# alpenlabs/dv-pari

Hardware: AMD Instinct MI355X
Metric: R1CS constraints/sec (prove) (higher is better)
Workload: dtype u32; 1 GPU; Proof::prove, synthetic dense R1CS, 2^20 constraints (BASELINE config #4); log2_constraints=20, n_wires=1048576, msm_pairs_per_proof=6291456, witness=resident in HBM, entry=dvp_prove_dev (Proof::prove with the witness resident), proofs_in_flight=1

## Files before the change

### dv-pari_amd/_native.py

```python
import ctypes as C
import os

import numpy as np

_HERE = os.path.dirname(os.path.abspath(__file__))
LIB_PATH = os.environ.get("DVP_LIB") or os.path.join(_HERE, "libdvpari_hip.so")

if not os.environ.get("DVP_NO_TORCH_PRELOAD"):
    try:
        import torch
    except Exception:
        pass

if not os.path.exists(LIB_PATH):
    raise ImportError(
        f"{LIB_PATH} is missing: build it with `python -c 'import __graft_entry__ as g; g.build()'` "
        "(hipcc --offload-arch=gfx950).  dv-pari_amd has no CPU fallback."
    )
lib = C.CDLL(LIB_PATH)

vp, u32, u64p, u8p, sz = C.c_void_p, C.c_uint32, C.c_void_p, C.c_void_p, C.c_size_t


class DlogReport(C.Structure):
# ... 158 lines not shown
    "dvp_prove_dev": (C.c_int, [vp, vp, u8p, vp]),
    "dvp_prove_begin": (C.c_int, [vp, vp, vp]),
    "dvp_prove_begin_partial": (C.c_int, [vp, vp, C.c_int, vp]),
    "dvp_prover_extend_count": (u32, [vp]),
    "dvp_prove_extend_vectors": (C.c_int, [vp, u32, vp]),
    "dvp_prover_extended_ptr": (C.c_int, [vp, u32, C.POINTER(vp)]),
    "dvp_prove_quotient": (C.c_int, [vp, vp]),
    "dvp_prove_mark_extended": (C.c_int, [vp, u32]),
    "dvp_prover_msm_size": (C.c_size_t, [vp, C.c_int]),
    "dvp_prover_msm_plan": (C.c_int, [vp, C.c_int, C.POINTER(C.c_int), C.POINTER(C.c_int)]),
    "dvp_prover_msm_table_bytes": (C.c_uint64, [vp, C.c_int, C.POINTER(C.c_int)]),
    "dvp_prover_set_table_budget": (C.c_int, [vp, C.c_uint64]),
    "dvp_prover_msm_coverage": (C.c_int, [vp, C.c_int, C.POINTER(C.c_size_t), C.POINTER(C.c_size_t), C.POINTER(C.c_int)]),
    "dvp_table_plan": (C.c_int, [sz, sz, C.c_uint64, C.POINTER(C.c_size_t * 2), C.POINTER(C.c_uint64 * 2)]),
    "dvp_aff_share_plan": (C.c_int, [C.c_longlong, u32, C.c_uint64, C.c_uint64, C.c_uint64]),
    "dvp_prover_msm_partial": (C.c_int, [vp, C.c_int, sz, sz, vp, vp, vp]),
    "dvp_prove_challenge": (C.c_int, [vp, vp, vp, vp]),
    "dvp_prove_challenge_partial": (C.c_int, [vp, vp, vp, C.c_size_t, C.c_size_t, C.c_size_t, C.c_size_t, vp, vp]),
    "dvp_prove_challenge_finish": (C.c_int, [vp, vp, C.c_uint32, C.c_size_t, C.c_size_t, vp]),
    "dvp_prove_finish": (C.c_int, [vp, vp, vp, u8p, vp]),
    "dvp_prover_debug_read": (C.c_int, [vp, C.c_char_p, u64p, sz]),
    "dvp_prover_debug_transcript_dev": (C.c_int, [vp, u8p, u64p, u32, u64p, u64p]),
    "dvp_prover_debug_force_alpha": (C.c_int, [vp, u64p]),
    "dvp_prover_domains": (C.c_int, [vp, u64p, u64p]),
    "dvp_prover_domain_tables": (C.c_int, [vp, C.c_int, u64p, u64p]),
    "dvp_ecfft_domain_tables": (C.c_int, [vp, C.c_int, u64p, u64p]),
    "dvp_file_fr_vec_write": (C.c_int, [C.c_char_p, u64p, sz]),
    "dvp_file_fr_vec_read": (C.c_int, [C.c_char_p, u64p, sz, C.POINTER(C.c_size_t)]),
    "dvp_file_point_vec_write": (C.c_int, [C.c_char_p, u8p, sz]),
    "dvp_file_point_vec_read": (C.c_int, [C.c_char_p, u8p, sz, C.POINTER(C.c_size_t)]),
# ... 144 lines not shown
```

### dv-pari_amd/csrc/capi.cpp

```cpp
#include "common.h"

#include <atomic>
#include <map>
#include <mutex>
#include <string>
#include <vector>
#include <cstring>
#include <cstdlib>
#include <climits>
#include <cxxabi.h>

namespace dvp {
thread_local int64_t g_last_error_index = -1;
thread_local hipError_t g_last_hip_error = hipSuccess;

bool g_prof_enabled = false;
static unsigned g_prof_mask = ~0u;
static std::mutex g_prof_mu;
static double g_prof_ms[PROF_NSLOTS] = {0};
static uint64_t g_prof_n[PROF_NSLOTS] = {0};
struct Pending { int slot; hipEvent_t e0, e1; uint64_t key; };
struct Shape { double ms = 0; uint64_t n = 0; };
static std::map<uint64_t, Shape> g_prof_round0;
static std::vector<Pending> g_prof_pending;
// ... 20 lines not shown
      g_prof_n[p.slot] += (p.slot == PROF_MSM_AFFINE_REST && p.key) ? p.key : 1;
      if (p.slot == PROF_MSM_ACCUM_AFFINE && p.key) { Shape& sh = g_prof_round0[p.key]; sh.ms += ms; sh.n += 1; }
    }
    (void)hipEventDestroy(p.e0);
    (void)hipEventDestroy(p.e1);
  }
  g_prof_pending.clear();
}

static std::atomic<uint64_t> g_host_waits[2];
void count_host_wait(int kind) { g_host_waits[kind & 1].fetch_add(1, std::memory_order_relaxed); }
static std::atomic<uint64_t> g_later_rounds[2];
void count_later_round(bool dense) { g_later_rounds[dense ? 1 : 0].fetch_add(1, std::memory_order_relaxed); }
static std::atomic<uint64_t> g_rounds_inv[2];
void count_round_inv(bool shared) { g_rounds_inv[shared ? 1 : 0].fetch_add(1, std::memory_order_relaxed); }

struct Census {
  std::mutex mu;
  std::map<std::string, LaunchCounter*> by_name;
};
static Census& census() {
  static Census* c = new Census;
  return *c;
}
LaunchCounter* census_register(const char* file, const char* tag_type) {
  int st = 0;
  char* dm = abi::__cxa_demangle(tag_type ? tag_type : "", nullptr, nullptr, &st);
  std::string v = (st == 0 && dm) ? dm : (tag_type ? tag_type : "");
  free(dm);
  for (size_t at; (at = v.find("(anonymous namespace)::")) != std::string::npos;) v.erase(at, 23);
// ... 43 lines not shown
    {"DVP_MSM_AFF_BMIN", &Tune::msm_aff_bmin},
    {"DVP_MSM_AFF_SHARE_INV", &Tune::msm_aff_share_inv},
    {"DVP_MSM_AFF_SHARE_MIN", &Tune::msm_aff_share_min},
    {"DVP_MSM_AFF_BMAX", &Tune::msm_aff_bmax},
    {"DVP_ECFFT_RADIX4", &Tune::ecfft_radix4},
    {"DVP_ECFFT_FOLD", &Tune::ecfft_fold},
    {"DVP_MSM_ACCUM_FAST", &Tune::msm_accum_fast},
    {"DVP_MSM_TAIL_GROUPS", &Tune::msm_tail_groups},
    {"DVP_MSM_ACCUM_HEX_MAX", &Tune::msm_accum_hex_max},
    {"DVP_GF_INV_TABS", &Tune::gf_inv_tabs},
    {"DVP_MSM_ACCUM_QUAD_MAX", &Tune::msm_accum_quad_max},
    {"DVP_MSM_BUCKET_PAIRS_MAX", &Tune::msm_bucket_pairs_max},
    {"DVP_MSM_SORT_FUSED", &Tune::msm_sort_fused},
    {"DVP_MSM_ROUND_PIPELINE", &Tune::msm_round_pipeline},
    {"DVP_MSM_ROUND_DENSE", &Tune::msm_round_dense},
    {"DVP_MSM_HEX_MAX", &Tune::msm_hex_max},
    {"DVP_MSM_QUAD_MAX", &Tune::msm_quad_max},
    {"DVP_MSM_FIXED_MIN", &Tune::msm_fixed_min},
    {"DVP_FR_BI_SHAPE", &Tune::fr_bi_shape},
    {"DVP_HORNER_MAX_PUB", &Tune::horner_max_pub},
    {"DVP_PROVE_HOST_TRANSCRIPT", &Tune::prove_host_transcript},
    {"DVP_TABLE_BUDGET_BYTES", &Tune::table_budget_bytes},
    {"DVP_MSM_TABLE_REFUSE", &Tune::msm_table_refuse},
    {"DVP_POINTS_MUL_W", &Tune::points_mul_w},
    {"DVP_MSM_SEG_PIECE", &Tune::msm_seg_piece},
    {"DVP_CIRCUIT_HASH_WINDOW", &Tune::circuit_hash_window},
    {"DVP_MSM_ALIGNED_SIGNED", &Tune::msm_aligned_signed},
    {"DVP_FR_DIGEST_WINDOW", &Tune::fr_digest_window},
};
static_assert(sizeof(Tune) == sizeof(kKnobs) / sizeof(kKnobs[0]) * sizeof(long long), "every field of Tune needs exactly one row of kKnobs");
// ... 54 lines not shown
extern "C" void dvp_profile_enable(int on) {
  dvp::g_prof_mask = on == 2 ? (1u << dvp::PROF_MSM_ACCUM_AFFINE) : ~0u;
  dvp::g_prof_enabled = on != 0;
}
extern "C" void dvp_profile_reset(void) {
  dvp::prof_collect();
  std::lock_guard<std::mutex> g(dvp::g_prof_mu);
  for (int i = 0; i < dvp::PROF_NSLOTS; ++i) { dvp::g_prof_ms[i] = 0; dvp::g_prof_n[i] = 0; }
  dvp::g_prof_round0.clear();
  dvp::g_host_waits[0] = 0;
  dvp::g_host_waits[1] = 0;
  dvp::g_later_rounds[0] = 0;
  dvp::g_later_rounds[1] = 0;
  dvp::g_rounds_inv[0] = 0;
  dvp::g_rounds_inv[1] = 0;
  dvp::Census& c = dvp::census();
  std::lock_guard<std::mutex> gc(c.mu);
  for (auto& e : c.by_name) e.second->n.store(0, std::memory_order_relaxed);
}
extern "C" int dvp_debug_launch_names(char* buf, size_t cap) {
  dvp::Census& c = dvp::census();
  std::lock_guard<std::mutex> g(c.mu);
  std::string all;
  for (auto& e : c.by_name) { all += e.first; all += '\n'; }
  if (buf && cap) {
    const size_t k = all.size() < cap - 1 ? all.size() : cap - 1;
    memcpy(buf, all.data(), k);
    buf[k] = 0;
  }
  return (int)(all.size() + 1);
// ... 12 lines not shown
extern "C" int dvp_profile_read(const char* name, double* total_ms, uint64_t* launches) {
  if (!name || !total_ms || !launches) return DVP_EINVAL;
  if (!strcmp(name, "host_waits_stream") || !strcmp(name, "host_waits_side")) {
    *total_ms = 0;
    *launches = dvp::g_host_waits[name[11] == 's' && name[12] == 'i' ? 1 : 0].load();
    return DVP_OK;
  }
  if (!strcmp(name, "later_rounds_word") || !strcmp(name, "later_rounds_dense")) {
    *total_ms = 0;
    *launches = dvp::g_later_rounds[name[13] == 'd' ? 1 : 0].load();
    return DVP_OK;
  }
  if (!strcmp(name, "rounds_inv_private") || !strcmp(name, "rounds_inv_shared")) {
    *total_ms = 0;
    *launches = dvp::g_rounds_inv[name[11] == 's' ? 1 : 0].load();
    return DVP_OK;
  }
  if (!strncmp(name, "launch:", 7)) {
    dvp::Census& c = dvp::census();
    std::lock_guard<std::mutex> g(c.mu);
    auto it = c.by_name.find(name + 7);
    if (it == c.by_name.end()) return DVP_EINVAL;
    *total_ms = 0;
    *launches = it->second->n.load(std::memory_order_relaxed);
    return DVP_OK;
  }
  dvp::prof_collect();
  std::lock_guard<std::mutex> g(dvp::g_prof_mu);
  for (int i = 0; i < dvp::PROF_NSLOTS; ++i)
    if (!strcmp(name, dvp::kProfNames[i])) { *total_ms = dvp::g_prof_ms[i]; *launches = dvp::g_prof_n[i]; return DVP_OK; }
// ... 46 lines not shown
```

### dv-pari_amd/csrc/common.h

```cpp
#pragma once
#include <hip/hip_runtime.h>
#include <stdint.h>
#include <stdio.h>
#include <string.h>

#include <algorithm>
#include <atomic>
#include <mutex>
#include <typeinfo>
#include <vector>

#include "../../include/dvpari_internal.h"
#include "fr.cuh"
#include "host_api.h"

namespace dvp {

extern thread_local hipError_t g_last_hip_error;

inline int hip_fail(hipError_t e, const char* what, const char* file, int line) {
  g_last_hip_error = e;
  fprintf(stderr, "[dvpari] HIP error %d (%s) at %s:%d: %s\n", (int)e, hipGetErrorString(e), file, line, what);
  if (e == hipErrorOutOfMemory) {
    (void)hipGetLastError();
// ... 179 lines not shown
  long long msm_aff_bmin = 8;
  long long msm_aff_share_inv = 2;
  long long msm_aff_share_min = 0;
  long long msm_aff_bmax = 136;
  long long ecfft_radix4 = 3;
  long long ecfft_fold = 1;
  long long msm_accum_fast = 1;
  long long msm_tail_groups = 1;
  long long msm_accum_hex_max = -1;
  long long gf_inv_tabs = 1;
  long long msm_accum_quad_max = 0;
  long long msm_bucket_pairs_max = 12;
  long long msm_sort_fused = 1;
  long long msm_round_pipeline = 2;
  long long msm_round_dense = 0;
  long long msm_hex_max = -1;
  long long msm_quad_max = 0;
  long long msm_fixed_min = 1ll << 16;
  long long fr_bi_shape = 6;
  long long horner_max_pub = -1;
  long long prove_host_transcript = 0;
  long long table_budget_bytes = -1;
  long long msm_table_refuse = 0;
  long long points_mul_w = 3;
  long long msm_seg_piece = 4;
  long long circuit_hash_window = 0;
  long long msm_aligned_signed = 1;
  long long fr_digest_window = 0;
};
Tune& tune();
// ... 5 lines not shown

enum ProfSlot { PROF_MSM_ACCUM_AFFINE = 0, PROF_MSM_TOTAL, PROF_EXTEND_TOTAL, PROF_PROVE_TOTAL, PROF_MSM_AFFINE_REST, PROF_MSM_SORT, PROF_MSM_TAIL, PROF_NSLOTS };
extern bool g_prof_enabled;
struct ProfScope {
  int slot;
  hipStream_t st;
  hipEvent_t e0 = nullptr, e1 = nullptr;
  uint64_t key = 0;
  ProfScope(int slot_, hipStream_t st_, uint64_t key_ = 0);
  void stop();
};
void prof_collect();
void count_host_wait(int kind);
void count_later_round(bool dense);
void count_round_inv(bool shared);

struct LaunchCounter {
  std::atomic<uint64_t> n{0};
};
LaunchCounter* census_register(const char* file, const char* tag_type);
template <auto K>
struct LaunchTag {};
template <auto K>
struct LaunchSite {
  static LaunchCounter* const counter;
};
template <auto K>
LaunchCounter* const LaunchSite<K>::counter = census_register(__BASE_FILE__, typeid(LaunchTag<K>).name());
template <auto K>
struct Launch;
// ... 11 lines not shown
```

### dv-pari_amd/csrc/msm.hip

```cpp
#include <algorithm>
#include <cstdlib>
#include <cstring>
#include <atomic>
#include <chrono>
#include <mutex>
#include <type_traits>
#include <vector>

#include "common.h"
#include "k233.cuh"
#include "tau.cuh"
#include "codec.cuh"
#include "host_api.h"
#include "msm_recode.cuh"
#include "msm_scan.cuh"
#include "msm_sort.cuh"
#include "msm_table.cuh"
#include "msm_reduce.cuh"
#include "msm_rounds.cuh"
#include "msm_merge.cuh"

namespace dvp {

static std::mutex g_wave_trace_mu;
// ... 235 lines not shown
  else if (per_key >= 8) f(std::integral_constant<int, 16>{});
  else f(std::integral_constant<int, 4>{});
}

struct MsmLayout {
  FxBits fb;
  bool fused1;
  uint32_t fx_S, fx_nblk, fx_nch;
  size_t sort_cells, affA_n, affB_n;
  bool affine_mode;
  size_t aff_min, e_est;
  int ra_plan;
  bool pipelined, side_stream;
  bool dense;
  size_t desc_at[41], desc_n;
  size_t rest_cap;
  uint32_t tail_groups;
  size_t bytes;
  bool sort_done_by_mscan() const { return pipelined && !side_stream; }
};
struct MsmBuffers {
  unsigned long long* err;
  uint32_t *d_max, *rest_n;
  uint16_t *digits, *plo, *hist16;
  uint32_t *digits32, *pid, *phist, *pbase, *ctot, *pstart, *cstart, *pcount, *chunk_off;
  uint32_t *cnt, *off, *ntask, *toff, *cnt2, *off2, *bsum, *items, *rest_list;
  Ld *bufA, *bufB, *bkt, *tail;
  Aff *affA, *affB;
  Gf* prefix;
  uint32_t* gdesc;
  uint32_t* rp;
  uint32_t* bsum2;
};
static MsmBuffers msm_carve(size_t n, const MsmPlan& p, const MsmFixedCtx* fx, const MsmLayout& L, void* base, size_t* bytes = nullptr) {
  Carver c{(uintptr_t)base};
  MsmBuffers b;
  const uint32_t FX_NP = L.fb.np();
  const size_t keys4 = ((size_t)p.nkeys + 1) * 4;
  b.err = c.take<unsigned long long>(32);
  b.d_max = (uint32_t*)(b.err + 1);
  b.rest_n = b.d_max + 1;
  b.digits = c.take<uint16_t>(fx ? 16 : (size_t)p.W * n * 2);
  b.digits32 = c.take<uint32_t>(fx && !L.fused1 ? p.e_max * 4 : 16);
// ... 1 lines not shown
  b.pid = c.take<uint32_t>(fx ? p.e_max * 4 : 16);
  for (uint32_t** r : {&b.phist, &b.pbase}) *r = c.take<uint32_t>(fx ? (size_t)L.fx_nblk * FX_NP * 4 : 16);
  b.ctot = c.take<uint32_t>(fx ? (size_t)FX_NP * L.fx_nch * 4 : 16);
  b.pstart = c.take<uint32_t>((FX_NP_MAX + 1) * 4 * 3);
  b.cstart = b.pstart + FX_NP_MAX + 1;
  b.pcount = b.cstart + FX_NP_MAX + 1;
  for (uint32_t** r : {&b.cnt, &b.off, &b.ntask, &b.toff, &b.cnt2, &b.off2}) *r = c.take<uint32_t>(keys4);
  b.bsum = c.take<uint32_t>(((size_t)p.nkeys / SCAN_BLK + 8) * 4);
  b.items = c.take<uint32_t>((p.e_max + (size_t)p.nkeys + 2) * 4);
  b.hist16 = c.take<uint16_t>(L.sort_cells * 2);
  b.chunk_off = c.take<uint32_t>(L.sort_cells * 4);
  b.bufA = c.take<Ld>(p.t1_max * sizeof(Ld));
  b.bufB = c.take<Ld>(p.t2_max * sizeof(Ld));
  b.affA = c.take<Aff>(L.affine_mode ? L.affA_n * sizeof(Aff) : 16);
  b.affB = c.take<Aff>(L.affine_mode ? L.affB_n * sizeof(Aff) : 16);
  b.prefix = c.take<Gf>(L.affine_mode ? (L.affA_n + 256) * sizeof(Gf) : 16);
  b.gdesc = c.take<uint32_t>(L.affine_mode ? L.desc_n * sizeof(uint32_t) : 16);
  b.rp = c.take<uint32_t>(L.pipelined ? (size_t)L.ra_plan * 2 * keys4 : 16);
  b.bsum2 = c.take<uint32_t>(((size_t)((L.ra_plan > 0 ? L.ra_plan : 1) + 1) * ((size_t)p.nkeys / SCAN_BLK + 1) + 8) * 4);
  b.bkt = c.take<Ld>((size_t)p.nkeys * sizeof(Ld));
  b.rest_list = c.take<uint32_t>(L.rest_cap * 4);
  b.tail = c.take<Ld>(((size_t)2 * p.W * p.c + 1 + 2 * (size_t)L.tail_groups) * sizeof(Ld));
  if (bytes) *bytes = c.o;
  return b;
}
static MsmLayout msm_layout(size_t n, const MsmPlan& p, const MsmFixedCtx* fx, const Tune& tn) {
  MsmLayout L{};
  L.fb = fx ? fx->bits() : FxBits{0, 0};
  L.fused1 = fx && fx->signed_digits && tn.msm_sort_fused != 0;
  L.fx_S = L.fused1 ? (FX_CHUNK / (uint32_t)p.W > 0 ? FX_CHUNK / (uint32_t)p.W : 1u) : 0u;
  L.fx_nblk = L.fused1 ? cdiv(n, L.fx_S) : cdiv(p.e_max, FX_CHUNK);
// ... 5 lines not shown
  L.aff_min = (size_t)(tn.msm_aff_min > 0 ? tn.msm_aff_min : 1);
  L.e_est = (size_t)n * (size_t)((fx && fx->signed_digits) ? p.W : (234 + p.c - 1) / p.c);
  while (L.affine_mode && L.ra_plan < 40 && (L.e_est >> (L.ra_plan + 1)) >= L.aff_min) ++L.ra_plan;
  L.pipelined = L.affine_mode && tn.msm_round_pipeline != 0 && L.ra_plan >= 2 && L.e_est >= 4 * (size_t)p.nkeys;
  L.side_stream = L.pipelined && tn.msm_round_pipeline == 1;
  L.dense = L.pipelined && tn.msm_round_dense != 0;
  L.desc_n = L.affA_n + 64;
  if (L.pipelined) {
    size_t cap_r = p.e_max + p.nkeys, at = 0;
    for (int r = 0; r < L.ra_plan; ++r) {
      const size_t out_max = cap_r / 2 + p.nkeys + 1;
      if (r >= 1) { L.desc_at[r] = at; at += (L.dense ? 2 : 1) * (out_max + 64); }
      cap_r = out_max;
    }
    if (at > L.desc_n) L.desc_n = at;
  }
  L.rest_cap = (size_t)p.nkeys + 2 + (p.e_max + (size_t)p.nkeys) / (size_t)(p.K > 0 ? p.K : 1);
  L.tail_groups = ((uint32_t)(p.W * p.c) + 15u) / 16u;
  (void)msm_carve(n, p, fx, L, nullptr, &L.bytes);
  return L;
}

static int msm_acquire_workspace(int dev, hipStream_t st, int ws_slots, size_t bytes, std::unique_lock<std::mutex>& g, MsmWorkspace** out) {
  int ws_slot = 0;
  for (int pass = 0; pass < 2 && !g.owns_lock(); ++pass)
    for (int sl = 0; sl < ws_slots && !g.owns_lock(); ++sl) {
      g = std::unique_lock<std::mutex>(g_ws_dev[dev][sl].mu, std::try_to_lock);
      if (g.owns_lock() && pass == 0 && g_ws_dev[dev][sl].busy_for(st)) g.unlock();
      if (g.owns_lock()) ws_slot = sl;
    }
// ... 207 lines not shown
    if (e != ~0ull) {
      g_last_error_index = (int64_t)(e & 0xffffffffull);
      return DVP_EINVAL;
    }
    return DVP_OK;
  }
};

static bool aff_share_plan(long long mode, uint32_t tpb, uint64_t planned, uint64_t share_min, uint64_t chip_full) {
  if (tpb != 128 && tpb != 256) return false;
  if (mode == 1) return true;
  if (mode != 2) return false;
  return planned >= (share_min ? share_min : chip_full);
}

struct PairRounds {
  const MsmRun& m;
  uint32_t *pc[3], *po[3];
  int cur = 0;
  const Aff* pts_in;
  size_t cap;
  int launched = 0, ra = 0;
  uint32_t max_cnt = 0;
  uint32_t aff_tpb = 0, aff_lds = 0, aff_cap = 0, aff_bmax_only = 0, aff_bmax = 0, aff_bmin = 0, wt_cap = 0;
  unsigned long long* wt_buf = nullptr;
  std::unique_lock<std::mutex> heavy;
  explicit PairRounds(const MsmRun& m_)
      : m(m_), pc{m_.b.cnt, m_.b.ntask, m_.b.cnt2}, po{m_.b.off, m_.b.toff, m_.b.off2}, pts_in(m_.bases0), cap(m_.p.e_max + m_.p.nkeys) {}
  uint32_t* rc(int r) const { return r == 0 ? m.b.cnt : m.b.rp + (size_t)(2 * (r - 1)) * ((size_t)m.p.nkeys + 1); }
  uint32_t* ro(int r) const { return r == 0 ? m.b.off : m.b.rp + (size_t)(2 * (r - 1) + 1) * ((size_t)m.p.nkeys + 1); }
// ... 36 lines not shown
    const size_t out_max = cap / 2 + nk + 1;
    Aff* outp = (r & 1) ? b.affB : b.affA;
    const uint32_t r_max = cdiv(cdiv(out_max, aff_cap), aff_bmax_only);
    const uint32_t grid = r_max * (aff_cap / aff_tpb) + 1;
    const bool share = aff_share_plan(m.tn.msm_aff_share_inv, aff_tpb, (uint64_t)(L.e_est >> (r + 1)),
                                      m.tn.msm_aff_share_min > 0 ? (uint64_t)m.tn.msm_aff_share_min : 0, (uint64_t)aff_cap * aff_bmin);
    const uint32_t bmax_arg = aff_bmax | (share ? AFF_SHARE_INV : 0u);
    ProfScope ps0(r == 0 ? PROF_MSM_ACCUM_AFFINE : -1, st, (uint64_t)m.n);
    WaveTrace wt{wt_buf, wt_cap, g_wave_trace_tag.fetch_add(wt_buf ? 1u : 0u)};
    with_bool(r == 0, [&](auto first) {
      with_bool(wt.buf != nullptr, [&](auto trace) {
        with_bool(r > 0 && L.dense, [&](auto dense) {
          constexpr bool FIRST = decltype(first)::value, TRACE = decltype(trace)::value, DENSE = decltype(dense)::value;
          if constexpr (!(FIRST && DENSE))
            DVP_LAUNCH((k_affine_round<FIRST, TRACE, DENSE>), dim3(grid), dim3(aff_tpb), aff_lds, st, pts_in, (const uint2*)(const void*)dsc, d_total,
                       aff_cap, bmax_arg, m.Tsq, b.prefix, outp, FIRST ? m.sign_mask : 0u, wt);
        });
      });
    });
    ps0.stop();
    if (r > 0) count_later_round(L.dense);
    count_round_inv(share);
    if (MsmCapture* c = m.cap; c && r < (int)CAPTURE_MAX_ROUNDS) {
      const bool dense_r = r > 0 && L.dense;
      const size_t pts_n = std::min(out_max, (r & 1) ? L.affB_n : L.affA_n);
      const size_t desc_n = r == 0 ? 0 : (L.pipelined ? (dense_r ? 2 : 1) * (out_max + 64) : std::min(out_max, L.desc_n));
      MsmCapture::Round& cr = c->rounds[r];
      cr.ocnt = c->grab(L.pipelined ? rc(r + 1) : pc[nxt], (size_t)nk * 4, st);
      cr.ooff = c->grab(L.pipelined ? ro(r + 1) : po[nxt], ((size_t)nk + 1) * 4, st);
      cr.desc = c->grab(dsc, desc_n * 4, st);
      cr.pts = c->grab(outp, pts_n * sizeof(Aff), st);
      c->hdr[CH_SHARE + r] = share ? 1u : 0u;
      c->nrounds = (uint32_t)r + 1;
    }
    pts_in = outp;
    cap = out_max;
    if (!L.pipelined) cur = nxt;
    return DVP_OK;
  }
  int begin() {
    const MsmLayout& L = m.L;
    if (m.ws_slots > 1 && L.affine_mode) {
      HeavyGate& hg = g_heavy[m.dev];
      heavy = std::unique_lock<std::mutex>(hg.mu);
      if (hg.last && hg.last != m.ws->ev_heavy) DVP_HIP(hipStreamWaitEvent(m.st, hg.last, 0));
    }
    if (L.affine_mode && (L.e_est >> 1) >= L.aff_min && L.e_est >= 4 * (size_t)m.p.nkeys) {
      DVP_TRY(run(0));
      launched = 1;
    }
    DVP_HIP(hipStreamSynchronize(m.ws->aux));
    count_host_wait(launched ? 1 : 0);
    max_cnt = *m.ws->pinned;
    if (L.affine_mode)
// ... 9 lines not shown
  int finish() {
    int r_evt = -1;
    if (heavy.owns_lock() && ra > 0) {
      const size_t gate_min = m.tn.msm_gate_min > 0 ? (size_t)m.tn.msm_gate_min : 1;
      r_evt = 0;
      while (r_evt + 1 < ra && (m.L.e_est >> (r_evt + 2)) >= gate_min) ++r_evt;
    }
    if (r_evt >= 0 && r_evt < launched) DVP_TRY(gate_event());
    int r = launched;
    if (r == 0 && ra > 0) {
      DVP_TRY(run(0));
      if (r_evt == 0) DVP_TRY(gate_event());
      r = 1;
    }
    ProfScope ps_rest(ra > r ? PROF_MSM_AFFINE_REST : -1, m.st, (uint64_t)(ra > r ? ra - r : 0));
    for (; r < ra; ++r) {
      DVP_TRY(run(r));
      if (r == r_evt) DVP_TRY(gate_event());
    }
    ps_rest.stop();
    if (m.L.pipelined) {
      pc[0] = rc(ra);
      po[0] = ro(ra);
      cur = 0;
    }
    if (heavy.owns_lock()) heavy.unlock();
    return DVP_OK;
  }
};

// ... 235 lines not shown
}
void msm_fixed_destroy(MsmFixedCtx* c) {
  if (!c) return;
  if (c->table) (void)hipFree(c->table);
  delete c;
}
int msm_fixed_dev(const MsmFixedCtx* c, const void* d_scalars, const void* d_inf, uint32_t lo, uint32_t hi, const MsmOut& out, hipStream_t st) {
  if (!c || lo > hi || hi > c->n_total) return DVP_EINVAL;
  return msm_core(d_scalars, nullptr, d_inf, hi - lo, c, lo, out, st);
}

}

using namespace dvp;

extern "C" int dvp_aff_share_plan(long long mode, uint32_t tpb, uint64_t planned, uint64_t share_min, uint64_t chip_full) {
  return aff_share_plan(mode, tpb, planned, share_min, chip_full) ? 1 : 0;
}

static size_t table_max_prefix(size_t total, uint64_t budget, size_t fixed_min, uint64_t* bytes) {
  *bytes = 0;
  if (total == 0 || total < fixed_min || total >= ((size_t)1 << 27)) return 0;
  size_t n = total;
  for (int it = 0; it < 64 && n > 0; ++it) {
    const uint64_t per = (uint64_t)msm_fixed_rows_for(n) * sizeof(Aff);
    const uint64_t fit = budget / per;
    if (fit >= n) break;
    n = (size_t)fit;
  }
  while (n > 0 && (uint64_t)msm_fixed_rows_for(n) * n * sizeof(Aff) > budget) --n;
// ... 111 lines not shown
```

### dv-pari_amd/csrc/msm_rounds.cuh

```cuda
#pragma once
#include "common.h"
#include "k233.cuh"
#include "msm_scan.cuh"
#include "msm_reduce.cuh"

namespace dvp {

constexpr uint32_t AFF_NONE = 0xffffffffu;
constexpr uint32_t DESC_PAIR = 0x80000000u;

__global__ void __launch_bounds__(256)
k_post_sort(uint32_t* __restrict__ items, const uint32_t* __restrict__ cnt, const uint32_t* __restrict__ off , uint32_t nkeys,
            uint32_t* __restrict__ ocnt, uint32_t* __restrict__ ooff , uint32_t* __restrict__ d_max) {
  const uint32_t k = blockIdx.x * blockDim.x + threadIdx.x;
  uint32_t m = 0;
  if (k <= nkeys) {
    const uint32_t o = off[k];
    ooff[k] = o >> 1;
    if (k < nkeys) {
      const uint32_t c = cnt[k];
      if (c & 1) items[o + c] = AFF_NONE;
      ocnt[k] = (c + 1) >> 1;
      m = c;
    }
// ... 166 lines not shown
    case 1: __builtin_amdgcn_s_setprio(1); break;
    default: __builtin_amdgcn_s_setprio(2); break;
  }
}
constexpr uint32_t AFF_BMAX = 136;
__device__ __forceinline__ uint32_t aff_slots_per_thread(uint32_t total, uint32_t cap, uint32_t bmax_bmin) {
  const uint32_t bmax = bmax_bmin & 0xffu, bmin = (bmax_bmin >> 8) & 0xffu;
  const uint32_t units = (total + cap - 1) / cap;
  const uint32_t R = (units + bmax - 1) / bmax;
  const uint32_t B = R ? (units + R - 1) / R : 1;
  return B < bmin ? bmin : B;
}
constexpr uint32_t AFF_SHARE_INV = 1u << 16;
constexpr uint32_t AFF_X_SLOT_BYTES = 2048;
constexpr uint32_t aff_exchange_bytes(uint32_t waves) { return waves == 4 ? 6 * AFF_X_SLOT_BYTES : waves == 2 ? 3 * AFF_X_SLOT_BYTES : 0; }
constexpr uint32_t AFF_INV_SPREAD = 256;
__device__ __forceinline__ void aff_x_put(uint32_t lane_addr, uint32_t slot, const Gf& v) {
  const uint32_t a = lane_addr + slot * AFF_X_SLOT_BYTES;
  gf_lds_st(a, (gf_u32x4){v.w[0], v.w[1], v.w[2], v.w[3]});
  gf_lds_st(a + 1024, (gf_u32x4){v.w[4], v.w[5], v.w[6], v.w[7]});
}
__device__ __forceinline__ Gf aff_x_get(uint32_t lane_addr, uint32_t slot) {
  const uint32_t a = lane_addr + slot * AFF_X_SLOT_BYTES;
  const gf_u32x4 lo = gf_lds_ld(a), hi = gf_lds_ld(a + 1024);
  Gf r;
  r.w[0] = lo.x; r.w[1] = lo.y; r.w[2] = lo.z; r.w[3] = lo.w;
  r.w[4] = hi.x; r.w[5] = hi.y; r.w[6] = hi.z; r.w[7] = hi.w;
  return r;
}
struct WaveTrace {
// ... 14 lines not shown
    for (int i = 0; i < 8; ++i) y.w[i] = gf_andxor(neg, x.w[i], y.w[i]);
  }
}
template <bool FIRST, bool DENSE>
__device__ __forceinline__ AffSlot aff_ld_desc(const uint2* __restrict__ desc, int k, int B, uint32_t sk, uint32_t lim) {
  const bool ok = k >= 0 && k < B && sk < lim;
  const uint32_t at = ok ? sk : 0u;
  const uint2 d = (FIRST || DENSE) ? desc[at] : make_uint2(((const uint32_t*)desc)[at], 0u);
  if (FIRST) return AffSlot{ok ? d.x : AFF_NONE, ok ? d.y : AFF_NONE, 0u};
  const uint32_t a = d.x & ~DESC_PAIR;
  return AffSlot{ok ? a : AFF_NONE, (ok && (d.x & DESC_PAIR)) ? a + 1 : AFF_NONE, d.y};
}
template <bool FIRST, bool TRACE = false, bool DENSE = false>
__global__ void __launch_bounds__(EC_TPB) __attribute__((amdgpu_waves_per_eu(3, 3)))
k_affine_round(const Aff* __restrict__ pts, const uint2* __restrict__ desc, const uint32_t* __restrict__ total_ptr ,
               uint32_t cap, uint32_t bmax, GfSqrTables T, Gf* __restrict__ prefix, Aff* __restrict__ out, uint32_t sign_mask, WaveTrace wt) {
  extern __shared__ char lds_raw[];
  unsigned long long tr_t0 = 0, tr_c0 = 0, tr_t1 = 0, tr_t2 = 0;
  uint32_t tr_inverted = 0;
  if (TRACE) { tr_t0 = wall_clock64(); tr_c0 = clock64(); }
  GfLdsK L = gf_ldsk_init(lds_raw);
#if AFF_PRIO
  const uint32_t wslot = __builtin_amdgcn_s_getreg(((4 - 1) << 11) | 4);
#endif
  const uint32_t sm = FIRST ? sign_mask : 0u;
  auto ldx = [&](uint32_t v) -> Gf { return pts[v & ~sm].x; };
  auto ldp = [&](uint32_t v, Gf& x, Gf& y) { aff_ld_point<FIRST>(pts, sm, v, x, y); };
  const uint32_t total = *total_ptr;
  const int B = (int)aff_slots_per_thread(total, cap, bmax);
  const uint32_t nthr = (total + B - 1) / B;
  const uint32_t tid = blockIdx.x * blockDim.x + threadIdx.x;
  const bool share = (bmax & AFF_SHARE_INV) != 0 && blockDim.x > 64;
  if (share ? blockIdx.x * blockDim.x >= nthr : tid >= nthr) return;
  const bool wave_live = __builtin_amdgcn_readfirstlane(tid & ~63u) < nthr;
  const uint32_t lim = tid < nthr ? total : 0u;
  auto ld_desc = [&](int k, uint32_t sk) -> AffSlot { return aff_ld_desc<FIRST, DENSE>(desc, k, B, sk, lim); };
  const Gf one = gf_one();
  Gf run = one;
  if (wave_live) {
    uint32_t sk = tid, sp = tid;
    AffSlot d0 = ld_desc(0, sk);
    sk += nthr;
    AffSlot d1 = ld_desc(1, sk);
    sk += nthr;
    Gf xa, ya, xb, yb;
    {
      const bool p = d0.b != AFF_NONE;
      ldp(p ? d0.a : 0u, xa, ya);
      ldp(p ? d0.b : 0u, xb, yb);
    }
#pragma unroll 1
    for (int k = 0; k < B; ++k) {
#if AFF_PRIO
      aff_set_prio(wslot + (uint32_t)k);
#endif
      const bool pair = d0.b != AFF_NONE;
      Gf den = gf_add(xa, xb), num = gf_add(ya, yb);
      const bool ainf = aff_or8(xa) == 0u, binf = aff_or8(xb) == 0u;
      const bool rare = pair & (ainf | binf | (aff_or8(den) == 0u));
      bool dbl = false;
      den.w[0] |= pair ? 0u : 1u;
      if (__any(rare)) {
        if (rare) {
          dbl = !ainf & !binf & (aff_or8(num) == 0u);
          den = dbl ? xa : one;
          num = dbl ? ya : gf_zero();
        }
      }
      const AffSlot d2 = ld_desc(k + 2, sk);
      sk += nthr;
      {
        const bool p = d1.b != AFF_NONE;
        if (!DENSE || __any(p)) {
          ldp(p ? d1.a : 0u, xa, ya);
          ldp(p ? d1.b : 0u, xb, yb);
        }
      }
      if (!DENSE || __any(pair)) {
        Gf np, nrun;
        gf_mul2(num, den, run, L, np, nrun);
        if (__any(rare)) {
          if (rare) np.w[7] |= dbl ? AFF_W7_DBL : AFF_W7_SKIP;
        }
        if (pair) prefix[sp] = np;
        run = nrun;
      }
      sp += nthr;
      d0 = d1;
      d1 = d2;
    }
// ... 4 lines not shown
  const uint32_t inverting = (blockIdx.x / AFF_INV_SPREAD) & (W - 1);
  Gf inv = run;
  if (share) {
    if (TRACE) tr_inverted = w == inverting ? 3u : 2u;
    aff_x_put(xa, w, run);
    __syncthreads();
    if (W == 4) {
      if ((w & 1u) == 0) aff_x_put(xa, 4 + (w >> 1), gf_mul(run, aff_x_get(xa, w + 1), L));
      __syncthreads();
    }
    if (w == inverting) {
      __builtin_amdgcn_s_setprio(3);
      inv = gf_mul(aff_x_get(xa, W == 4 ? 4 : 0), aff_x_get(xa, W == 4 ? 5 : 1), L);
    }
  }
  if (!share || w == inverting) inv = gf_inv_fast(inv, T, L);
  if (share) {
    if (w == inverting) {
      if (W == 4) {
        Gf ia, ib;
        gf_mul2(aff_x_get(xa, 5), aff_x_get(xa, 4), inv, L, ia, ib);
        aff_x_put(xa, 4, ia);
        aff_x_put(xa, 5, ib);
      } else {
        aff_x_put(xa, 2, inv);
      }
      __builtin_amdgcn_s_setprio(0);
    }
    __syncthreads();
    inv = gf_mul(aff_x_get(xa, W == 4 ? 4 + (w >> 1) : 2), aff_x_get(xa, w ^ 1u), L);
  }
  if (TRACE) tr_t2 = wall_clock64();
  if (wave_live) {
    uint32_t sp = (uint32_t)(B - 1) * nthr + tid, sk = sp;
    auto ld_slot = [&](const AffSlot& e, uint32_t s, Gf& x1, Gf& y1, Gf& x2, Gf& pre) {
      const bool pair = e.b != AFF_NONE;
      ldp(e.a != AFF_NONE ? e.a : 0u, x1, y1);
      x2 = ldx(pair ? e.b : 0u);
      pre = prefix[pair ? s : 0u];
    };
    AffSlot e0 = ld_desc(B - 1, sk);
    sk -= nthr;
    AffSlot e1 = ld_desc(B - 2, sk);
    sk -= nthr;
    Gf px, py, qx, pre;
    ld_slot(e0, sp, px, py, qx, pre);
#pragma unroll 1
    for (int k = B - 1; k >= 0; --k) {
#if AFF_PRIO
      aff_set_prio(wslot + (uint32_t)k);
#endif
      const bool pair = e0.b != AFF_NONE, flagged = pair & (pre.w[7] > AFF_W7_MASK);
      const uint32_t sidx = DENSE ? e0.o : sp;
// ... 36 lines not shown
      } else if (e0.a != AFF_NONE && !pair) {
        out[sidx].x = px;
        out[sidx].y = py;
      }
      sp -= nthr;
      e0 = e1;
      e1 = e2;
      px = npx;
      py = npy;
      pre = npre;
    }
  }
#if AFF_PRIO
  __builtin_amdgcn_s_setprio(0);
#endif
  if (TRACE) {
    const unsigned long long t3 = wall_clock64(), c3 = clock64();
    if ((threadIdx.x & 63u) == 0) {
      const unsigned long long i = atomicAdd(wt.buf, 1ull);
      if (i < wt.cap) {
        unsigned long long* r = wt.buf + 8 + 8 * i;
        r[0] = tr_t0; r[1] = tr_t1; r[2] = tr_t2; r[3] = t3;
        r[4] = tr_c0; r[5] = c3;
        r[6] = (unsigned long long)__builtin_amdgcn_s_getreg((31 << 11) | 4) | ((unsigned long long)__builtin_amdgcn_s_getreg((31 << 11) | 20) << 32);
        r[7] = (unsigned long long)blockIdx.x | ((unsigned long long)wt.tag << 32) | ((unsigned long long)(uint32_t)B << 48) | ((unsigned long long)(threadIdx.x >> 6) << 56) |
               ((unsigned long long)tr_inverted << 60);
      }
    }
  }
}
// ... 38 lines not shown
```

### include/dvpari_internal.h

```cpp
#ifndef DVPARI_INTERNAL_H
#define DVPARI_INTERNAL_H

#include "dvpari.h"

#ifdef __cplusplus
extern "C" {
#endif

int dvp_tune_set(const char* name, long long value);
int dvp_tune_get(const char* name, long long* value);
void dvp_tune_reset(void);

void dvp_profile_enable(int on);
void dvp_profile_reset(void);
int dvp_profile_read(const char* name, double* total_ms, uint64_t* launches);
int dvp_debug_launch_names(char* buf, size_t cap);
int dvp_debug_msm_rest_len(uint32_t* n);

int dvp_debug_msm_capture_arm(size_t arena_bytes);
int dvp_debug_msm_capture_fetch(void* out, size_t cap_bytes, size_t* need);
int dvp_debug_msm_enc(dvp_msm_ctx* ctx, const uint64_t* scalars, const uint64_t* bases_xy, size_t lo, size_t hi, uint64_t out_xy[8],
                      int* out_is_infinity, uint8_t out_enc[30]);

int dvp_profile_round0_shapes(uint64_t* pairs, double* total_ms, uint64_t* launches, int cap);

int dvp_ubench_gf_mul(int reps, double* products_per_s);
int dvp_ubench_fr_mul(int reps, double* muladds_per_s);
int dvp_ubench_points_check(const void* d_xy, const void* d_inf, const void* d_enc, size_t n, void* d_scratch, int reps,
                            double* check_ms, double* decode_ms);
int dvp_ubench_points_mul(const void* d_scalars, const void* d_xy, size_t n, void* d_scratch, int reps, double* mul_ms, double* mulgen_ms);
int dvp_debug_wave_trace(void* d_buf, uint32_t n_records);
int dvp_ubench_gather(const void* d_table, size_t table_bytes, int reps, double* gathers_per_s);
int dvp_prover_msm_table_ptr(const dvp_prover* p, int which, const void** d_table, uint64_t* bytes);

int dvp_table_plan(size_t size0, size_t size1, uint64_t budget_bytes, size_t covered[2], uint64_t bytes[2]);

int dvp_aff_share_plan(long long mode, uint32_t tpb, uint64_t planned, uint64_t share_min, uint64_t chip_full);

int dvp_debug_recode_signed(const uint64_t* scalars, size_t n, int c_bits, uint32_t* out_words, int* windows);

int dvp_debug_recode_tnaf(const uint64_t* scalars, size_t n, int w, int8_t* digits, int* n_digits, int32_t* alpha );

int dvp_setup_scalars(const uint64_t tau[4], const uint64_t delta[4], const uint64_t epsilon[4], uint32_t log2_m, uint32_t n_public,
                      uint32_t n_rows, uint32_t n_wires, const uint64_t* coeffs, uint32_t n_coeffs, const uint32_t* const row_ptr[3],
                      const uint32_t* const wire_ids[3], const uint32_t* const coeff_ids[3], uint64_t* out_scalars, size_t out_cap);

int dvp_setup_cache_dir_ex(const uint64_t tau[4], const uint64_t delta[4], const uint64_t epsilon[4], const char* cache_dir,
                           uint32_t n_public, int write_precomputes, uint64_t* out_scalars, size_t out_cap, uint32_t* out_n_wires,
                           uint32_t* out_log2_m);

int dvp_prover_debug_transcript_dev(dvp_prover* p, const uint8_t commit_p[30], const uint64_t* public_inputs, uint32_t n_public,
                                    uint64_t out_alpha[4], uint64_t out_neg_z_alpha[4]);
// ... 90 lines not shown
```

Before: 59.75 million constraints/s.

## Fuse later affine MSM reduction rounds into one persistent kernel launch

Adds a fused path that runs all remaining affine bucket-reduction rounds inside a single k_affine_round launch. Each workgroup takes a key range found by binary search over the round offsets and loops through the rounds, with only block-level barriers and fences between rounds. This is meant to remove per-round launch overhead and the grid-wide serialization between small later rounds. It relies on each workgroup's key range staying self-contained across rounds, uses an extra output buffer, and may load-balance poorly when buckets are skewed.

```diff
diff --git a/dv-pari_amd/_native.py b/dv-pari_amd/_native.py
--- a/dv-pari_amd/_native.py
+++ b/dv-pari_amd/_native.py
@@ -196,6 +196,7 @@
     "dvp_prover_msm_coverage": (C.c_int, [vp, C.c_int, C.POINTER(C.c_size_t), C.POINTER(C.c_size_t), C.POINTER(C.c_int)]),
     "dvp_table_plan": (C.c_int, [sz, sz, C.c_uint64, C.POINTER(C.c_size_t * 2), C.POINTER(C.c_uint64 * 2)]),
     "dvp_aff_share_plan": (C.c_int, [C.c_longlong, u32, C.c_uint64, C.c_uint64, C.c_uint64]),
+    "dvp_round_fuse_plan": (C.c_int, [C.c_longlong, C.c_int, C.c_int, C.c_int, C.c_uint64, C.c_uint64, C.c_uint64]),
     "dvp_prover_msm_partial": (C.c_int, [vp, C.c_int, sz, sz, vp, vp, vp]),
     "dvp_prove_challenge": (C.c_int, [vp, vp, vp, vp]),
     "dvp_prove_challenge_partial": (C.c_int, [vp, vp, vp, C.c_size_t, C.c_size_t, C.c_size_t, C.c_size_t, vp, vp]),
diff --git a/dv-pari_amd/csrc/capi.cpp b/dv-pari_amd/csrc/capi.cpp
--- a/dv-pari_amd/csrc/capi.cpp
+++ b/dv-pari_amd/csrc/capi.cpp
@@ -58,6 +58,8 @@
 void count_later_round(bool dense) { g_later_rounds[dense ? 1 : 0].fetch_add(1, std::memory_order_relaxed); }
 static std::atomic<uint64_t> g_rounds_inv[2];
 void count_round_inv(bool shared) { g_rounds_inv[shared ? 1 : 0].fetch_add(1, std::memory_order_relaxed); }
+static std::atomic<uint64_t> g_rounds_fused;
+void count_round_fused() { g_rounds_fused.fetch_add(1, std::memory_order_relaxed); }
 
 struct Census {
   std::mutex mu;
@@ -131,6 +133,9 @@
     {"DVP_MSM_SORT_FUSED", &Tune::msm_sort_fused},
     {"DVP_MSM_ROUND_PIPELINE", &Tune::msm_round_pipeline},
     {"DVP_MSM_ROUND_DENSE", &Tune::msm_round_dense},
+    {"DVP_MSM_ROUND_FUSED", &Tune::msm_round_fused},
+    {"DVP_MSM_ROUND_FUSED_MIN", &Tune::msm_round_fused_min},
+    {"DVP_MSM_ROUND_FUSED_WGS", &Tune::msm_round_fused_wgs},
     {"DVP_MSM_HEX_MAX", &Tune::msm_hex_max},
     {"DVP_MSM_QUAD_MAX", &Tune::msm_quad_max},
     {"DVP_MSM_FIXED_MIN", &Tune::msm_fixed_min},
@@ -215,6 +220,7 @@
   dvp::g_later_rounds[1] = 0;
   dvp::g_rounds_inv[0] = 0;
   dvp::g_rounds_inv[1] = 0;
+  dvp::g_rounds_fused = 0;
   dvp::Census& c = dvp::census();
   std::lock_guard<std::mutex> gc(c.mu);
   for (auto& e : c.by_name) e.second->n.store(0, std::memory_order_relaxed);
@@ -257,6 +263,11 @@
   if (!strcmp(name, "rounds_inv_private") || !strcmp(name, "rounds_inv_shared")) {
     *total_ms = 0;
     *launches = dvp::g_rounds_inv[name[11] == 's' ? 1 : 0].load();
+    return DVP_OK;
+  }
+  if (!strcmp(name, "rounds_fused")) {
+    *total_ms = 0;
+    *launches = dvp::g_rounds_fused.load();
     return DVP_OK;
   }
   if (!strncmp(name, "launch:", 7)) {
diff --git a/dv-pari_amd/csrc/common.h b/dv-pari_amd/csrc/common.h
--- a/dv-pari_amd/csrc/common.h
+++ b/dv-pari_amd/csrc/common.h
@@ -217,6 +217,9 @@
   long long msm_sort_fused = 1;
   long long msm_round_pipeline = 2;
   long long msm_round_dense = 0;
+  long long msm_round_fused = 2;
+  long long msm_round_fused_min = 0;
+  long long msm_round_fused_wgs = 0;
   long long msm_hex_max = -1;
   long long msm_quad_max = 0;
   long long msm_fixed_min = 1ll << 16;
@@ -252,6 +255,7 @@
 void count_host_wait(int kind);
 void count_later_round(bool dense);
 void count_round_inv(bool shared);
+void count_round_fused();
 
 struct LaunchCounter {
   std::atomic<uint64_t> n{0};
diff --git a/dv-pari_amd/csrc/msm.hip b/dv-pari_amd/csrc/msm.hip
--- a/dv-pari_amd/csrc/msm.hip
+++ b/dv-pari_amd/csrc/msm.hip
@@ -273,6 +273,8 @@
   bool pipelined, side_stream;
   bool dense;
   size_t desc_at[41], desc_n;
+  bool fusable;
+  size_t fused_at[41], fused_n;
   size_t rest_cap;
   uint32_t tail_groups;
   size_t bytes;
@@ -285,7 +287,7 @@
   uint32_t *digits32, *pid, *phist, *pbase, *ctot, *pstart, *cstart, *pcount, *chunk_off;
   uint32_t *cnt, *off, *ntask, *toff, *cnt2, *off2, *bsum, *items, *rest_list;
   Ld *bufA, *bufB, *bkt, *tail;
-  Aff *affA, *affB;
+  Aff *affA, *affB, *affF;
   Gf* prefix;
   uint32_t* gdesc;
   uint32_t* rp;
@@ -317,7 +319,8 @@
   b.bufB = c.take<Ld>(p.t2_max * sizeof(Ld));
   b.affA = c.take<Aff>(L.affine_mode ? L.affA_n * sizeof(Aff) : 16);
   b.affB = c.take<Aff>(L.affine_mode ? L.affB_n * sizeof(Aff) : 16);
-  b.prefix = c.take<Gf>(L.affine_mode ? (L.affA_n + 256) * sizeof(Gf) : 16);
+  b.prefix = c.take<Gf>(L.affine_mode ? (std::max(L.affA_n, L.fused_n) + 256) * sizeof(Gf) : 16);
+  b.affF = c.take<Aff>(L.fusable ? L.fused_n * sizeof(Aff) : 16);
   b.gdesc = c.take<uint32_t>(L.affine_mode ? L.desc_n * sizeof(uint32_t) : 16);
   b.rp = c.take<uint32_t>(L.pipelined ? (size_t)L.ra_plan * 2 * keys4 : 16);
   b.bsum2 = c.take<uint32_t>(((size_t)((L.ra_plan > 0 ? L.ra_plan : 1) + 1) * ((size_t)p.nkeys / SCAN_BLK + 1) + 8) * 4);
@@ -353,6 +356,17 @@
       cap_r = out_max;
     }
     if (at > L.desc_n) L.desc_n = at;
+  }
+  L.fusable = L.pipelined && !L.dense && L.ra_plan >= 3 &&
+              (tn.msm_round_fused == 1 || (tn.msm_round_fused == 2 && (L.e_est >> 2) >= (tn.msm_round_fused_min > 0 ? (size_t)tn.msm_round_fused_min : (size_t)1 << 16)));
+  if (L.fusable) {
+    size_t cap_r = p.e_max + p.nkeys, at = 0;
+    for (int r = 0; r < L.ra_plan; ++r) {
+      const size_t out_max = cap_r / 2 + p.nkeys + 1;
+      if (r >= 1) { L.fused_at[r] = at; at += (out_max + 64 + 3) & ~(size_t)3; }
+      cap_r = out_max;
+    }
+    L.fused_n = at;
   }
   L.rest_cap = (size_t)p.nkeys + 2 + (p.e_max + (size_t)p.nkeys) / (size_t)(p.K > 0 ? p.K : 1);
   L.tail_groups = ((uint32_t)(p.W * p.c) + 15u) / 16u;
@@ -590,6 +604,13 @@
   return planned >= (share_min ? share_min : chip_full);
 }
 
+static bool round_fuse_plan(long long mode, bool layout_ok, bool traced, int remaining, uint64_t planned, uint64_t fused_min, uint64_t chip_full) {
+  if (!layout_ok || traced || remaining < 2) return false;
+  if (mode == 1) return true;
+  if (mode != 2) return false;
+  return planned >= (fused_min ? fused_min : chip_full);
+}
+
 struct PairRounds {
   const MsmRun& m;
   uint32_t *pc[3], *po[3];
@@ -656,7 +677,7 @@
           constexpr bool FIRST = decltype(first)::value, TRACE = decltype(trace)::value, DENSE = decltype(dense)::value;
           if constexpr (!(FIRST && DENSE))
             DVP_LAUNCH((k_affine_round<FIRST, TRACE, DENSE>), dim3(grid), dim3(aff_tpb), aff_lds, st, pts_in, (const uint2*)(const void*)dsc, d_total,
-                       aff_cap, bmax_arg, m.Tsq, b.prefix, outp, FIRST ? m.sign_mask : 0u, wt);
+                       aff_cap, bmax_arg, m.Tsq, b.prefix, outp, FIRST ? m.sign_mask : 0u, wt, AffFused{});
         });
       });
     });
@@ -680,6 +701,46 @@
     if (!L.pipelined) cur = nxt;
     return DVP_OK;
   }
+  int run_fused(int r0, uint32_t wgs) {
+    const MsmLayout& L = m.L;
+    const MsmBuffers& b = m.b;
+    const uint32_t nk = m.p.nkeys;
+    hipStream_t st = m.st;
+    AffFused fz{};
+    fz.rp = b.rp;
+    fz.out = b.affF;
+    fz.nkeys = nk;
+    fz.r_begin = (uint32_t)r0;
+    fz.r_end = (uint32_t)ra;
+    for (int r = r0; r < ra; ++r) {
+      const bool share = aff_share_plan(m.tn.msm_aff_share_inv, aff_tpb, (uint64_t)(L.e_est >> (r + 1)),
+                                        m.tn.msm_aff_share_min > 0 ? (uint64_t)m.tn.msm_aff_share_min : 0, (uint64_t)aff_cap * aff_bmin);
+      if (share) fz.share_mask |= 1ull << r;
+      fz.desc_at[r] = L.desc_at[r];
+      fz.out_at[r] = fz.pre_at[r] = L.fused_at[r];
+      count_later_round(false);
+      count_round_inv(share);
+      count_round_fused();
+    }
+    const WaveTrace wt{nullptr, 0, 0};
+    DVP_LAUNCH((k_affine_round<false, false, false>), dim3(wgs), dim3(aff_tpb), aff_lds, st, pts_in, (const uint2*)(const void*)b.gdesc, ro(r0 + 1) + nk,
+               aff_cap, aff_bmax | AFF_FUSED, m.Tsq, b.prefix, b.affF, 0u, wt, fz);
+    for (int r = r0; r < ra; ++r) {
+      const size_t out_max = cap / 2 + nk + 1;
+      if (MsmCapture* c = m.cap; c && r < (int)CAPTURE_MAX_ROUNDS) {
+        MsmCapture::Round& cr = c->rounds[r];
+        cr.ocnt = c->grab(rc(r + 1), (size_t)nk * 4, st);
+        cr.ooff = c->grab(ro(r + 1), ((size_t)nk + 1) * 4, st);
+        cr.desc = c->grab(b.gdesc + L.desc_at[r], (out_max + 64) * 4, st);
+        cr.pts = c->grab(b.affF + L.fused_at[r], std::min(out_max, (r & 1) ? L.affB_n : L.affA_n) * sizeof(Aff), st);
+        c->hdr[CH_SHARE + r] = (fz.share_mask >> r) & 1ull ? 1u : 0u;
+        c->nrounds = (uint32_t)r + 1;
+      }
+      pts_in = b.affF + L.fused_at[r];
+      cap = out_max;
+    }
+    return DVP_OK;
+  }
   int begin() {
     const MsmLayout& L = m.L;
     if (m.ws_slots > 1 && L.affine_mode) {
@@ -719,6 +780,14 @@
       r = 1;
     }
     ProfScope ps_rest(ra > r ? PROF_MSM_AFFINE_REST : -1, m.st, (uint64_t)(ra > r ? ra - r : 0));
+    const uint32_t chip_wgs = aff_cap / aff_tpb;
+    const uint32_t fused_wgs = m.tn.msm_round_fused_wgs > 0 ? (uint32_t)std::min<long long>(m.tn.msm_round_fused_wgs, 1 << 20) : chip_wgs;
+    if (r >= 1 && round_fuse_plan(m.tn.msm_round_fused, m.L.fusable, wt_buf != nullptr, ra - r, (uint64_t)(m.L.e_est >> (r + 1)),
+                                  m.tn.msm_round_fused_min > 0 ? (uint64_t)m.tn.msm_round_fused_min : 0, (uint64_t)aff_cap * aff_bmin)) {
+      DVP_TRY(run_fused(r, fused_wgs));
+      if (r_evt >= r) DVP_TRY(gate_event());
+      r = ra;
+    }
     for (; r < ra; ++r) {
       DVP_TRY(run(r));
       if (r == r_evt) DVP_TRY(gate_event());
@@ -984,6 +1053,9 @@
 
 using namespace dvp;
 
+extern "C" int dvp_round_fuse_plan(long long mode, int layout_ok, int traced, int remaining, uint64_t planned, uint64_t fused_min, uint64_t chip_full) {
+  return round_fuse_plan(mode, layout_ok != 0, traced != 0, remaining, planned, fused_min, chip_full) ? 1 : 0;
+}
 extern "C" int dvp_aff_share_plan(long long mode, uint32_t tpb, uint64_t planned, uint64_t share_min, uint64_t chip_full) {
   return aff_share_plan(mode, tpb, planned, share_min, chip_full) ? 1 : 0;
 }
diff --git a/dv-pari_amd/csrc/msm_rounds.cuh b/dv-pari_amd/csrc/msm_rounds.cuh
--- a/dv-pari_amd/csrc/msm_rounds.cuh
+++ b/dv-pari_amd/csrc/msm_rounds.cuh
@@ -204,6 +204,23 @@
 constexpr uint32_t AFF_SHARE_INV = 1u << 16;
 constexpr uint32_t AFF_X_SLOT_BYTES = 2048;
 constexpr uint32_t aff_exchange_bytes(uint32_t waves) { return waves == 4 ? 6 * AFF_X_SLOT_BYTES : waves == 2 ? 3 * AFF_X_SLOT_BYTES : 0; }
+constexpr uint32_t AFF_FUSED = 1u << 17;
+constexpr int AFF_FUSED_MAX = 40;
+struct AffFused {
+  const uint32_t* rp;
+  Aff* out;
+  uint32_t nkeys, r_begin, r_end;
+  unsigned long long share_mask;
+  unsigned long long desc_at[AFF_FUSED_MAX], out_at[AFF_FUSED_MAX], pre_at[AFF_FUSED_MAX];
+};
+__device__ __forceinline__ uint32_t aff_range_cut(const uint32_t* __restrict__ o, uint32_t nkeys, uint32_t target) {
+  uint32_t lo = 0, hi = nkeys;
+  while (lo < hi) {
+    const uint32_t mid = lo + ((hi - lo) >> 1);
+    if (o[mid] < target) lo = mid + 1; else hi = mid;
+  }
+  return lo;
+}
 constexpr uint32_t AFF_INV_SPREAD = 256;
 __device__ __forceinline__ void aff_x_put(uint32_t lane_addr, uint32_t slot, const Gf& v) {
   const uint32_t a = lane_addr + slot * AFF_X_SLOT_BYTES;
@@ -248,7 +265,8 @@
 template <bool FIRST, bool TRACE = false, bool DENSE = false>
 __global__ void __launch_bounds__(EC_TPB) __attribute__((amdgpu_waves_per_eu(3, 3)))
 k_affine_round(const Aff* __restrict__ pts, const uint2* __restrict__ desc, const uint32_t* __restrict__ total_ptr ,
-               uint32_t cap, uint32_t bmax, GfSqrTables T, Gf* __restrict__ prefix, Aff* __restrict__ out, uint32_t sign_mask, WaveTrace wt) {
+               uint32_t cap, uint32_t bmax, GfSqrTables T, Gf* __restrict__ prefix, Aff* __restrict__ out, uint32_t sign_mask, WaveTrace wt,
+               AffFused fz) {
   extern __shared__ char lds_raw[];
   unsigned long long tr_t0 = 0, tr_c0 = 0, tr_t1 = 0, tr_t2 = 0;
   uint32_t tr_inverted = 0;
@@ -260,19 +278,54 @@
   const uint32_t sm = FIRST ? sign_mask : 0u;
   auto ldx = [&](uint32_t v) -> Gf { return pts[v & ~sm].x; };
   auto ldp = [&](uint32_t v, Gf& x, Gf& y) { aff_ld_point<FIRST>(pts, sm, v, x, y); };
-  const uint32_t total = *total_ptr;
-  const int B = (int)aff_slots_per_thread(total, cap, bmax);
-  const uint32_t nthr = (total + B - 1) / B;
-  const uint32_t tid = blockIdx.x * blockDim.x + threadIdx.x;
-  const bool share = (bmax & AFF_SHARE_INV) != 0 && blockDim.x > 64;
-  if (share ? blockIdx.x * blockDim.x >= nthr : tid >= nthr) return;
+  const bool fused = !FIRST && !TRACE && !DENSE && (bmax & AFF_FUSED) != 0;
+  const size_t ostride = (size_t)fz.nkeys + 1;
+  uint32_t k0 = 0, k1 = 0, rnd = 0, r_end = 1;
+  if (fused) {
+    rnd = fz.r_begin;
+    r_end = fz.r_end;
+    const uint32_t* o = fz.rp + (size_t)(2 * rnd + 1) * ostride;
+    const uint32_t tot = o[fz.nkeys];
+    k0 = aff_range_cut(o, fz.nkeys, (uint32_t)((unsigned long long)tot * blockIdx.x / gridDim.x));
+    k1 = blockIdx.x + 1 == gridDim.x ? fz.nkeys : aff_range_cut(o, fz.nkeys, (uint32_t)((unsigned long long)tot * (blockIdx.x + 1) / gridDim.x));
+    if (o[k0] == o[k1]) return;
+  }
+  const Gf one = gf_one();
+  const uint2* const desc0 = desc;
+  Gf* const prefix0 = prefix;
+  int B = 0;
+#pragma unroll 1
+  for (;;) {
+  uint32_t start = 0, idle = 0, total, nthr, tid;
+  bool share;
+  if (fused) {
+    const uint32_t* o = fz.rp + (size_t)(2 * rnd + 1) * ostride;
+    start = o[k0];
+    idle = (o - 2 * ostride)[k0];
+    const uint32_t len = o[k1] - start, bmin = (bmax >> 8) & 0xffu;
+    const uint32_t need = (len + blockDim.x - 1) / blockDim.x;
+    B = (int)(need < bmin ? bmin : need);
+    nthr = (len + B - 1) / B;
+    total = start + len;
+    tid = threadIdx.x;
+    share = ((fz.share_mask >> rnd) & 1ull) != 0 && blockDim.x > 64;
+    desc = (const uint2*)((const uint32_t*)desc0 + fz.desc_at[rnd]);
+    prefix = prefix0 + fz.pre_at[rnd];
+    out = fz.out + fz.out_at[rnd];
+  } else {
+    total = *total_ptr;
+    B = (int)aff_slots_per_thread(total, cap, bmax);
+    nthr = (total + B - 1) / B;
+    tid = blockIdx.x * blockDim.x + threadIdx.x;
+    share = (bmax & AFF_SHARE_INV) != 0 && blockDim.x > 64;
+    if (share ? blockIdx.x * blockDim.x >= nthr : tid >= nthr) return;
+  }
   const bool wave_live = __builtin_amdgcn_readfirstlane(tid & ~63u) < nthr;
   const uint32_t lim = tid < nthr ? total : 0u;
   auto ld_desc = [&](int k, uint32_t sk) -> AffSlot { return aff_ld_desc<FIRST, DENSE>(desc, k, B, sk, lim); };
-  const Gf one = gf_one();
   Gf run = one;
   if (wave_live) {
-    uint32_t sk = tid, sp = tid;
+    uint32_t sk = start + tid, sp = sk;
     AffSlot d0 = ld_desc(0, sk);
     sk += nthr;
     AffSlot d1 = ld_desc(1, sk);
@@ -280,8 +333,8 @@
     Gf xa, ya, xb, yb;
     {
       const bool p = d0.b != AFF_NONE;
-      ldp(p ? d0.a : 0u, xa, ya);
-      ldp(p ? d0.b : 0u, xb, yb);
+      ldp(p ? d0.a : idle, xa, ya);
+      ldp(p ? d0.b : idle, xb, yb);
     }
 #pragma unroll 1
     for (int k = 0; k < B; ++k) {
@@ -306,8 +359,8 @@
       {
         const bool p = d1.b != AFF_NONE;
         if (!DENSE || __any(p)) {
-          ldp(p ? d1.a : 0u, xa, ya);
-          ldp(p ? d1.b : 0u, xb, yb);
+          ldp(p ? d1.a : idle, xa, ya);
+          ldp(p ? d1.b : idle, xb, yb);
         }
       }
       if (!DENSE || __any(pair)) {
@@ -342,7 +395,7 @@
       inv = gf_mul(aff_x_get(xa, W == 4 ? 4 : 0), aff_x_get(xa, W == 4 ? 5 : 1), L);
     }
   }
-  if (!share || w == inverting) inv = gf_inv_fast(inv, T, L);
+  if (share ? w == inverting : wave_live) inv = gf_inv_fast(inv, T, L);
   if (share) {
     if (w == inverting) {
       if (W == 4) {
@@ -360,11 +413,11 @@
   }
   if (TRACE) tr_t2 = wall_clock64();
   if (wave_live) {
-    uint32_t sp = (uint32_t)(B - 1) * nthr + tid, sk = sp;
+    uint32_t sp = start + (uint32_t)(B - 1) * nthr + tid, sk = sp;
     auto ld_slot = [&](const AffSlot& e, uint32_t s, Gf& x1, Gf& y1, Gf& x2, Gf& pre) {
       const bool pair = e.b != AFF_NONE;
-      ldp(e.a != AFF_NONE ? e.a : 0u, x1, y1);
-      x2 = ldx(pair ? e.b : 0u);
+      ldp(e.a != AFF_NONE ? e.a : idle, x1, y1);
+      x2 = ldx(pair ? e.b : idle);
       pre = prefix[pair ? s : 0u];
     };
     AffSlot e0 = ld_desc(B - 1, sk);
@@ -431,6 +484,12 @@
 #if AFF_PRIO
   __builtin_amdgcn_s_setprio(0);
 #endif
+  if (++rnd >= r_end) break;
+  pts = out;
+  __builtin_amdgcn_fence(__ATOMIC_RELEASE, "agent");
+  __syncthreads();
+  __builtin_amdgcn_fence(__ATOMIC_ACQUIRE, "agent");
+  }
   if (TRACE) {
     const unsigned long long t3 = wall_clock64(), c3 = clock64();
     if ((threadIdx.x & 63u) == 0) {
diff --git a/include/dvpari_internal.h b/include/dvpari_internal.h
--- a/include/dvpari_internal.h
+++ b/include/dvpari_internal.h
@@ -36,6 +36,8 @@
 int dvp_table_plan(size_t size0, size_t size1, uint64_t budget_bytes, size_t covered[2], uint64_t bytes[2]);
 
 int dvp_aff_share_plan(long long mode, uint32_t tpb, uint64_t planned, uint64_t share_min, uint64_t chip_full);
+
+int dvp_round_fuse_plan(long long mode, int layout_ok, int traced, int remaining, uint64_t planned, uint64_t fused_min, uint64_t chip_full);
 
 int dvp_debug_recode_signed(const uint64_t* scalars, size_t n, int c_bits, uint32_t* out_words, int* windows);
 
```

New measurement: 56.58 million constraints/s. -5.3%, worse.
